# hieunghia-pat/OpenViIC

Hardware: AMD Instinct MI355X
Metric: captions/sec (whole node) at beam=5, 50 regions x d2048 (higher is better)
Workload: dtype f32; 1 GPU; standard_transformer beam=5, B=256 per GPU, 50x2048 synthetic regions, V=10201, max_len=20, random-init weights; global_batch=256, parallelism=dp1, streams=4

## Files before the change

### openviic_amd/csrc/gemm.hip

```cpp
#include <atomic>
#include <type_traits>
#include <mutex>
#include <vector>

#include <hip/hip_ext.h>

#include "common.h"
#include "dropout.h"

namespace {


#ifndef OVC_F32_BUFS
#define OVC_F32_BUFS 1
#endif
template <int BM, int BN, int WM, int WN, int WK, int BK, int NC>
struct TileConfig {
    static constexpr int LDT = BK + 4;
    static constexpr int kThreads = 256;
    static constexpr int kWaveM = BM / WM;
    static constexpr int kWaveN = BN / WN;
    static constexpr int TM = kWaveM / 32;
    static constexpr int TN = kWaveN / 32;
    static constexpr int kLoadA = BM * (BK / 4) / kThreads;
    static constexpr int kLoadB = BN * (BK / 4) / kThreads;
    static constexpr int kChains = NC * WK;
    static constexpr int kBufs = OVC_F32_BUFS;
    static constexpr int kTileFloats = kBufs * (BM + BN) * LDT;
    static constexpr int kRedFloats = (WK - 1) * NC * BM * BN;
    static constexpr int kLdsFloats = kTileFloats > kRedFloats ? kTileFloats : kRedFloats;
    static_assert(WM * WN * WK == 4, "four waves per workgroup");
    static_assert(kChains == 1 || kChains == 4, "K-order classes: one chain or four");
    static_assert(BK % 8 == 0 && (kChains == 1 || BK % 32 == 0), "a K tile holds whole 8-deep groups (four chains: whole 4-group periods)");
    static_assert(kWaveM % 32 == 0 && kWaveN % 32 == 0, "wave tile must be a multiple of 32x32");
    static_assert(kLoadA >= 1 && kLoadB >= 1, "tile too small for 256 loader threads");

};

__device__ __forceinline__ int xcd_remap(int bid, int nwg) {
    const int xcd = bid & 7, q = nwg >> 3, r = nwg & 7;
    const int base = xcd < r ? xcd * (q + 1) : r * (q + 1) + (xcd - r) * q;
    return base + (bid >> 3);
}

__device__ __forceinline__ void tile_coords(int tiles_m, int group_m, int xcd_pm, int& tile_m, int& tile_n_all) {
    const int nwg = gridDim.x;
    const int tile = xcd_remap(blockIdx.x, nwg);
    const int tiles_n_all = nwg / tiles_m;
    if (xcd_pm > 0) {
        const int per_chunk = nwg >> 3, chunk = tile / per_chunk, j = tile - chunk * per_chunk;
        const int sub_m = tiles_m / xcd_pm, cm = chunk % xcd_pm, cn = chunk / xcd_pm;
        const int sub_n = tiles_n_all / (8 / xcd_pm);
        tile_m = cm * sub_m + j % sub_m;
        tile_n_all = cn * sub_n + j / sub_m;
    } else {
        const int group_size = group_m * tiles_n_all;
        const int group = tile / group_size;
        const int first_m = group * group_m;
        const int gm = min(group_m, tiles_m - first_m);
        const int in_group = tile - group * group_size;
        tile_n_all = in_group / gm;
        tile_m = first_m + (in_group - tile_n_all * gm);
    }
}

struct TileMap {
    int nwg, tiles_m, tiles_n_all, tiles_n_per_seg;
    int xcd_pm, pm_shift, sub_m, sub_n;
    unsigned sub_m_magic, seg_magic;
    int group_m, group_size, gm_last;
    unsigned group_size_magic, group_m_magic, gm_last_magic;
    int kslice;
};

__device__ __forceinline__ int fast_div(int x, unsigned magic, int d) {
    if (d == 1) return x;
    const unsigned q = __umulhi((unsigned)x, magic);
    return (int)(q * (unsigned)d > (unsigned)x ? q - 1 : q);
}

__device__ __forceinline__ void tile_coords_fast(const TileMap& t, int bid, int& tile_m, int& tile_n_all) {
    const int xcd = bid & 7, q = t.nwg >> 3, r = t.nwg & 7;
    if (t.xcd_pm > 0) {
        const int j = bid >> 3;
        const int cm = xcd & (t.xcd_pm - 1), cn = xcd >> t.pm_shift;
        const int jq = fast_div(j, t.sub_m_magic, t.sub_m);
        tile_m = cm * t.sub_m + (j - jq * t.sub_m);
        tile_n_all = cn * t.sub_n + jq;
    } else {
        const int base = xcd < r ? xcd * (q + 1) : r * (q + 1) + (xcd - r) * q;
        const int tile = base + (bid >> 3);
        const int group = fast_div(tile, t.group_size_magic, t.group_size);
        const int first_m = group * t.group_m;
        const int in_group = tile - group * t.group_size;
        const bool last = first_m + t.group_m > t.tiles_m;
        const int gm = last ? t.gm_last : t.group_m;
        tile_n_all = last ? fast_div(in_group, t.gm_last_magic, t.gm_last) : fast_div(in_group, t.group_m_magic, t.group_m);
        tile_m = first_m + (in_group - tile_n_all * gm);
    }
}

template <int TM, int TN, bool kDrop = false>
__device__ __forceinline__ void store_wave_tiles(const GemmArgs& p, const float* __restrict__ bias, float* __restrict__ Cseg,
                                                 const f32x16 (&acc)[TM][TN], int m0, int n0, int lane,
                                                 const DropoutSite& drop = DropoutSite{}) {
    float* __restrict__ C = Cseg + (size_t)blockIdx.y * p.part_stride;
    uint64_t drop_seed = 0;
    if constexpr (kDrop) drop_seed = (uint64_t)*drop.seed;
    const int half = lane >> 5;
    const bool has_res = p.R != nullptr;
    const __amdgpu_buffer_rsrc_t rsrc_c = __builtin_amdgcn_make_buffer_rsrc(C, 0, p.M * p.ldc * 4, 0x00020000);
    const __amdgpu_buffer_rsrc_t rsrc_r = __builtin_amdgcn_make_buffer_rsrc(const_cast<float*>(has_res ? p.R : p.A1), 0,
                                                                             has_res && p.res_mod == 0 ? p.M * p.ldr * 4 : 0, 0x00020000);
    constexpr int kOutOfRange = 0x7ffffff0;
#pragma unroll
    for (int j = 0; j < TN; ++j) {
        const int n = n0 + j * 32 + (lane & 31);
        const bool n_ok = n < p.seg_n;
        const float bv = bias ? bias[min(n, p.seg_n - 1)] : 0.f;
#pragma unroll
        for (int i = 0; i < TM; ++i) {
            const int mbase = m0 + i * 32 + 4 * half;
            float out[16];
#pragma unroll
            for (int r = 0; r < 16; ++r) {
                const float v = acc[i][j][r] + bv;
                out[r] = p.act == 1 ? fmaxf(v, 0.f) : v;
            }
            if constexpr (kDrop) {
                uint32_t keep = 0;
#pragma unroll 1
                for (int r = 0; r < 16; ++r) {
                    const uint64_t row = (uint64_t)(mbase + (r & 3) + 8 * (r >> 2));
                    keep |= (ovc_dropout_keep(drop_seed, drop.site, row * (uint64_t)drop.cols + (uint64_t)n, drop.thr) ? 1u : 0u) << r;
                }
#pragma unroll
                for (int r = 0; r < 16; ++r) out[r] = (keep >> r) & 1u ? out[r] * drop.scale : 0.f;
            }
            if (has_res) {
                float res[16];
                if (p.res_mod == 0) {
                    const int voff_r = n_ok ? (mbase * p.ldr + n) * 4 : kOutOfRange;
#pragma unroll
                    for (int r = 0; r < 16; ++r)
                        res[r] = __builtin_bit_cast(float, __builtin_amdgcn_raw_buffer_load_b32(rsrc_r, voff_r, ((r & 3) + 8 * (r >> 2)) * p.ldr * 4, 0));
                } else {
#pragma unroll
                    for (int r = 0; r < 16; ++r) {
                        const int mc = min(mbase + (r & 3) + 8 * (r >> 2), p.M - 1) % p.res_mod;
                        res[r] = p.R[(size_t)mc * p.ldr + min(n, p.seg_n - 1)];
                    }
                }
#pragma unroll
                for (int r = 0; r < 16; ++r) out[r] += res[r];
            }
            const int voff_c = n_ok ? (mbase * p.ldc + n) * 4 : kOutOfRange;
#pragma unroll
            for (int r = 0; r < 16; ++r)
                __builtin_amdgcn_raw_buffer_store_b32(__builtin_bit_cast(int, out[r]), rsrc_c, voff_c, ((r & 3) + 8 * (r >> 2)) * p.ldc * 4, 0);
            if (p.stats_t) {
                const int mrow = m0 + i * 32 + 4 * half;
                float v[16];
                float bm = -INFINITY;
#pragma unroll
                for (int r = 0; r < 16; ++r) {
                    v[r] = mrow + (r & 3) + 8 * (r >> 2) < p.M ? out[r] : -INFINITY;
                    bm = fmaxf(bm, v[r]);
                }
                float x, y;
                ovc_swap_rows<true>(bm, x, y);
                bm = fmaxf(x, y);
                float bs = 0.f;
#pragma unroll
                for (int r = 0; r < 16; ++r) bs += __expf(v[r] - bm);
                ovc_swap_rows<true>(bs, x, y);
                bs = x + y;
                if (lane < 32 && n_ok && m0 + i * 32 < p.M)
                    *reinterpret_cast<f32x2*>(p.stats_t + 2 * ((size_t)n * p.stats_ld + ((m0 + i * 32) >> 5))) = f32x2{bm, bs};
            }
            if (p.stats) {
                float bm = 0.f, bs = 0.f;
#pragma unroll
                for (int r = 0; r < 16; ++r) {
                    const float v = n_ok ? out[r] : -INFINITY;
                    const float m = half_wave_max(v);
                    const float sum = half_wave_sum(__expf(v - m));
                    if ((lane & 15) == r) { bm = m; bs = sum; }
                }
                const int rr = lane & 15, row = mbase + (rr & 3) + 8 * (rr >> 2);
                if ((lane & 31) < 16 && row < p.M && n0 + j * 32 < p.seg_n)
                    *reinterpret_cast<f32x2*>(p.stats + 2 * ((size_t)row * p.stats_ld + ((n0 + j * 32) >> 5))) = f32x2{bm, bs};
            }
        }
    }
}

template <int TM, int TN>
__device__ __forceinline__ void store_wave_tiles_score(const GemmArgs& p, const float* __restrict__ bias, const f32x16 (&acc)[TM][TN],
                                                       int m0, int n0, int lane, const int32_t* __restrict__ tgt,
                                                       float* __restrict__ tgt_logit) {
    const int half = lane >> 5;
#pragma unroll
    for (int j = 0; j < TN; ++j) {
        const int n = n0 + j * 32 + (lane & 31);
        const bool n_ok = n < p.seg_n;
        const float bv = bias ? bias[min(n, p.seg_n - 1)] : 0.f;
        const int target = n_ok ? tgt[n] : -1;
#pragma unroll
        for (int i = 0; i < TM; ++i) {
            const int mbase = m0 + i * 32 + 4 * half;
            float out[16];
#pragma unroll
            for (int r = 0; r < 16; ++r) {
                const float v = acc[i][j][r] + bv;
                out[r] = p.act == 1 ? fmaxf(v, 0.f) : v;
            }
#pragma unroll
            for (int r = 0; r < 16; ++r)
                if (target - mbase == (r & 3) + 8 * (r >> 2)) tgt_logit[n] = out[r];
            const int mrow = m0 + i * 32 + 4 * half;
            float v[16];
            float bm = -INFINITY;
#pragma unroll
            for (int r = 0; r < 16; ++r) {
                v[r] = mrow + (r & 3) + 8 * (r >> 2) < p.M ? out[r] : -INFINITY;
                bm = fmaxf(bm, v[r]);
            }
            float x, y;
            ovc_swap_rows<true>(bm, x, y);
            bm = fmaxf(x, y);
            float bs = 0.f;
#pragma unroll
            for (int r = 0; r < 16; ++r) bs += __expf(v[r] - bm);
            ovc_swap_rows<true>(bs, x, y);
            bs = x + y;
            if (lane < 32 && n_ok && m0 + i * 32 < p.M)
                *reinterpret_cast<f32x2*>(p.stats_t + 2 * ((size_t)n * p.stats_ld + ((m0 + i * 32) >> 5))) = f32x2{bm, bs};
        }
    }
}

#include "gemm_split.h"
#include "gemm_rows16.h"

template <int BM, int BN, int BK, int NC>
constexpr int min_waves_per_simd() { return BM * BN <= 32 * 64 ? 5 : (BM * BN <= 64 * 64 ? (NC == 4 && BK == 64 ? 3 : 4) : 1); }

template <int BM, int BN, int WM, int WN, int WK, int BK, int NC>
__global__ __launch_bounds__(256, (min_waves_per_simd<BM, BN, BK, NC>())) void gemm_f32_mfma(TileMap tmap, GemmArgs p) {
#define OVC_GEMM_F32_EPILOGUE \
    store_wave_tiles<Cfg::TM, Cfg::TN>(p, seg_bias, seg_C, acc[0], m0 + wm * Cfg::kWaveM, n0 + wn * Cfg::kWaveN, lane)
#include "gemm_f32_body.inc"
#undef OVC_GEMM_F32_EPILOGUE
}

template <int BM, int BN, int WM, int WN, int WK, int BK, int NC>
__global__ __launch_bounds__(256, (min_waves_per_simd<BM, BN, BK, NC>())) void gemm_f32_mfma_gated(TileMap tmap, GemmArgs p,
                                                                                                 const int32_t* __restrict__ gate) {
    if (ovc_gate_closed(gate)) return;
#define OVC_GEMM_F32_EPILOGUE \
    store_wave_tiles<Cfg::TM, Cfg::TN>(p, seg_bias, seg_C, acc[0], m0 + wm * Cfg::kWaveM, n0 + wn * Cfg::kWaveN, lane)
#include "gemm_f32_body.inc"
#undef OVC_GEMM_F32_EPILOGUE
}

template <int BM, int BN, int WM, int WN, int WK, int BK, int NC>
__global__ __launch_bounds__(256, (min_waves_per_simd<BM, BN, BK, NC>())) void gemm_f32_mfma_dropout(TileMap tmap, GemmArgs p,
                                                                                                   DropoutSite drop) {
#define OVC_GEMM_F32_EPILOGUE \
    store_wave_tiles<Cfg::TM, Cfg::TN, true>(p, seg_bias, seg_C, acc[0], m0 + wm * Cfg::kWaveM, n0 + wn * Cfg::kWaveN, lane, drop)
#include "gemm_f32_body.inc"
#undef OVC_GEMM_F32_EPILOGUE
}

template <int BM, int BN, int WM, int WN, int WK, int BK, int NC>
__global__ __launch_bounds__(256, (min_waves_per_simd<BM, BN, BK, NC>())) void gemm_f32_mfma_score(TileMap tmap, GemmArgs p,
                                                                                                 const int32_t* tgt, float* tgt_logit) {
#define OVC_GEMM_F32_EPILOGUE \
    store_wave_tiles_score<Cfg::TM, Cfg::TN>(p, seg_bias, acc[0], m0 + wm * Cfg::kWaveM, n0 + wn * Cfg::kWaveN, lane, tgt, tgt_logit)
#include "gemm_f32_body.inc"
#undef OVC_GEMM_F32_EPILOGUE
}

enum TileOrderRegime { kOrderSuperRows = 0, kOrderSplitSmallA = 1, kOrderSplitLargeA = 2 };
int tile_order(const GemmArgs& a, int tiles_m, int tiles_n, int* group_m, int* xcd_pm) {
    const size_t a_bytes = sizeof(float) * (size_t)a.M * (a.K1 + a.K2);
    *group_m = a_bytes <= (size_t)3 << 20 ? tiles_m : (tiles_m < 8 ? tiles_m : 8);
    *xcd_pm = 0;
    const int slices = a.ksplit > 1 ? a.ksplit : 1;
    const size_t w_bytes = sizeof(float) * (size_t)a.seg_n * a.nseg * (a.K1 + a.K2);
    const int tiles_n_all = tiles_n * a.nseg;
    if (a_bytes / slices <= (size_t)3 << 20) {
        size_t best = 8 * a_bytes + w_bytes;
        for (int pm = 2; pm <= 8; pm *= 2) {
            if (tiles_m % pm || tiles_n_all % (8 / pm)) continue;
            const size_t cost = (size_t)(8 / pm) * a_bytes + (size_t)pm * w_bytes;
            if (cost < best) { best = cost; *xcd_pm = pm; }
        }
        if (*xcd_pm > 0) return kOrderSplitSmallA;
    } else if (slices == 1 && w_bytes <= (size_t)3 << 20) {
        size_t best = ~(size_t)0;
        for (int pm = 8; pm >= 2; pm /= 2) {
            if (tiles_m % pm || tiles_n_all % (8 / pm) || a_bytes / pm > (size_t)3 << 20) continue;
            const size_t cost = (size_t)(8 / pm) * a_bytes + (size_t)pm * w_bytes;
            if (cost < best) { best = cost; *xcd_pm = pm; }
        }
        if (*xcd_pm > 0) return kOrderSplitLargeA;
    }
    return kOrderSuperRows;
}

inline void tile_counts(const GemmArgs& a, int bm, int bn, int* tiles_m, int* tiles_n) {
    *tiles_m = (a.M + bm - 1) / bm;
    *tiles_n = (a.seg_n + bn - 1) / bn;
}

enum GemmInstance { kInstPlain = 0, kInstGated = 1, kInstDropout = 2, kInstScoring = 3, kInstPlanesDirect = 4 };
inline int f32_instance(const GemmLaunchOpts& opts) {
    return opts.tgt_logit ? kInstScoring : (opts.drop_seed ? kInstDropout : (opts.gate ? kInstGated : kInstPlain));
}
inline bool split_reads_planes(const GemmArgs& a, int bk) {
    bool planes = (a.K1 + a.K2) % bk == 0 && a.K1 % bk == 0;
    for (int s = 0; s < a.nseg; ++s) planes = planes && a.seg[s].Wp != nullptr;
    return planes;
}

TileMap make_tile_map(int nwg, int tiles_m, int tiles_n_per_seg, int group_m, int xcd_pm, int kslice) {
    auto magic = [](int d) { return d > 1 ? (unsigned)(((uint64_t)1 << 32) / (uint64_t)d + 1) : 0u; };
    TileMap t{};
    t.nwg = nwg; t.tiles_m = tiles_m; t.tiles_n_all = nwg / tiles_m; t.tiles_n_per_seg = tiles_n_per_seg;
// ... 613 lines not shown
```

### openviic_amd/csrc/gemm_f32_body.inc

```
    using Cfg = TileConfig<BM, BN, WM, WN, WK, BK, NC>;
    constexpr int LDT = Cfg::LDT;
    constexpr int kVecPerRow = BK / 4;
    constexpr int kRowsPerPass = 256 / kVecPerRow;
    extern __shared__ __attribute__((aligned(16))) float lds[];

    const int tid = threadIdx.x;
    const int lane = tid & 63;
    const int wave = tid >> 6;
    const int wk = wave / (WM * WN);
    const int wm = (wave / WN) % WM, wn = wave % WN;

    const TileMap t = tmap;
    const float* const a1_ptr = p.A1;
    const float* const w0_ptr = p.seg[0].W;
    const float* const bias0_ptr = p.seg[0].bias;
    float* const c0_ptr = p.seg[0].C;
    const float* const a2_shared = p.A2;
    uint8_t* const zero_rows_ptr = p.zero_rows_out;
    const int arg_lda1 = p.lda1, arg_lda2 = p.lda2, arg_K1 = p.K1, arg_K2 = p.K2, arg_M = p.M, arg_seg_n = p.seg_n, arg_nseg = p.nseg;
    asm volatile("" ::"s"(t.nwg), "s"(t.tiles_m), "s"(t.tiles_n_all), "s"(t.tiles_n_per_seg), "s"(t.xcd_pm), "s"(t.pm_shift), "s"(t.sub_m),
                 "s"(t.sub_n), "s"(t.sub_m_magic), "s"(t.seg_magic), "s"(t.group_m), "s"(t.group_size), "s"(t.gm_last),
                 "s"(t.group_size_magic), "s"(t.group_m_magic), "s"(t.gm_last_magic), "s"(t.kslice), "s"(a1_ptr), "s"(w0_ptr),
                 "s"(bias0_ptr), "s"(c0_ptr), "s"(arg_lda1), "s"(arg_K1), "s"(arg_K2), "s"(arg_M), "s"(arg_seg_n), "s"(arg_nseg),
                 "s"(a2_shared), "s"(zero_rows_ptr), "s"(arg_lda2), "s"(p.R), "s"(p.ldc), "s"(p.ldr), "s"(p.res_mod), "s"(p.act),
                 "s"(p.part_stride), "s"(p.stats), "s"(p.stats_t), "s"(p.stats_ld));

    int tile_m, tile_n_all;
    tile_coords_fast(t, (int)blockIdx.x, tile_m, tile_n_all);
    const int seg = arg_nseg == 1 ? 0 : fast_div(tile_n_all, t.seg_magic, t.tiles_n_per_seg);
    const int tile_n = tile_n_all - seg * t.tiles_n_per_seg;
    const int m0 = tile_m * BM, n0 = tile_n * BN;

    const float* __restrict__ W = arg_nseg == 1 ? w0_ptr : p.seg[seg].W;
    const float* __restrict__ seg_bias = arg_nseg == 1 ? bias0_ptr : p.seg[seg].bias;
    float* __restrict__ seg_C = arg_nseg == 1 ? c0_ptr : p.seg[seg].C;
    const int K = arg_K1 + arg_K2;
    const int kslice = t.kslice;
    const int kbase = (int)blockIdx.y * kslice;
    const int nkt = (kslice + BK - 1) / BK;

    constexpr int kBufFloats = (BM + BN) * LDT;

    f32x4 stage_a[Cfg::kLoadA], stage_b[Cfg::kLoadB];

    const bool k_tail = (K % BK) != 0 || (p.K1 % BK) != 0;
    bool a_ok = true, w_ok = true;

    const __amdgpu_buffer_rsrc_t rsrc_a1 = __builtin_amdgcn_make_buffer_rsrc(const_cast<float*>(a1_ptr), 0, arg_M * arg_lda1 * 4, 0x00020000);
    const float* a2 = arg_K2 ? (p.seg[seg].A2 ? p.seg[seg].A2 : a2_shared) : a1_ptr;
    const __amdgpu_buffer_rsrc_t rsrc_a2 = __builtin_amdgcn_make_buffer_rsrc(const_cast<float*>(a2), 0,
                                                                              arg_K2 ? arg_M * arg_lda2 * 4 : 0, 0x00020000);
    const __amdgpu_buffer_rsrc_t rsrc_w = __builtin_amdgcn_make_buffer_rsrc(const_cast<float*>(W), 0, arg_seg_n * K * 4, 0x00020000);
    int off_a1[Cfg::kLoadA], off_a2[Cfg::kLoadA], off_w[Cfg::kLoadB];
    {
        const int kq = tid % kVecPerRow;
#pragma unroll
        for (int i = 0; i < Cfg::kLoadA; ++i) {
            const int row = m0 + tid / kVecPerRow + i * kRowsPerPass;
            off_a1[i] = (row * arg_lda1 + kq * 4) * 4;
            off_a2[i] = (row * arg_lda2 + kq * 4) * 4;
        }
#pragma unroll
        for (int i = 0; i < Cfg::kLoadB; ++i) off_w[i] = ((n0 + tid / kVecPerRow + i * kRowsPerPass) * K + kq * 4) * 4;
    }
    auto load_tile = [&](int kt) {
        const int k0 = kbase + kt * BK;
        const bool second = k0 >= p.K1;
        if (k_tail) {
            const int kq = tid % kVecPerRow;
            a_ok = (second ? k0 - p.K1 : k0) + kq * 4 < (second ? p.K2 : p.K1);
            w_ok = k0 + kq * 4 < K;
        }
        if (!second) {
#pragma unroll
            for (int i = 0; i < Cfg::kLoadA; ++i)
                stage_a[i] = __builtin_bit_cast(f32x4, __builtin_amdgcn_raw_buffer_load_b128(rsrc_a1, off_a1[i], k0 * 4, 0));
        } else {
#pragma unroll
            for (int i = 0; i < Cfg::kLoadA; ++i)
                stage_a[i] = __builtin_bit_cast(f32x4, __builtin_amdgcn_raw_buffer_load_b128(rsrc_a2, off_a2[i], (k0 - p.K1) * 4, 0));
        }
#pragma unroll
        for (int i = 0; i < Cfg::kLoadB; ++i)
            stage_b[i] = __builtin_bit_cast(f32x4, __builtin_amdgcn_raw_buffer_load_b128(rsrc_w, off_w[i], k0 * 4, 0));
    };
    const bool row_sums = zero_rows_ptr != nullptr && tile_n_all == 0;
    float rs[Cfg::kLoadA];
#pragma unroll
    for (int i = 0; i < Cfg::kLoadA; ++i) rs[i] = 0.f;
    auto store_tile = [&](int buf) {
        const int kq = tid % kVecPerRow;
        if (k_tail) {
#pragma unroll
            for (int i = 0; i < Cfg::kLoadA; ++i)
                if (!a_ok) stage_a[i] = f32x4{0.f, 0.f, 0.f, 0.f};
#pragma unroll
            for (int i = 0; i < Cfg::kLoadB; ++i)
                if (!w_ok) stage_b[i] = f32x4{0.f, 0.f, 0.f, 0.f};
        }
        if (row_sums) {
#pragma unroll
            for (int i = 0; i < Cfg::kLoadA; ++i) rs[i] += (stage_a[i][0] + stage_a[i][1]) + (stage_a[i][2] + stage_a[i][3]);
        }
#pragma unroll
        for (int i = 0; i < Cfg::kLoadA; ++i) {
            const int row = tid / kVecPerRow + i * kRowsPerPass;
            *reinterpret_cast<f32x4*>(lds + buf * kBufFloats + row * LDT + kq * 4) = stage_a[i];
        }
#pragma unroll
        for (int i = 0; i < Cfg::kLoadB; ++i) {
            const int row = tid / kVecPerRow + i * kRowsPerPass;
            *reinterpret_cast<f32x4*>(lds + buf * kBufFloats + (BM + row) * LDT + kq * 4) = stage_b[i];
        }
    };

    f32x16 acc[NC][Cfg::TM][Cfg::TN];
#pragma unroll
    for (int c = 0; c < NC; ++c)
#pragma unroll
        for (int i = 0; i < Cfg::TM; ++i)
#pragma unroll
            for (int j = 0; j < Cfg::TN; ++j)
#pragma unroll
                for (int r = 0; r < 16; ++r) acc[c][i][j][r] = 0.f;

    const int frag_row = lane & 31;
    const int frag_k = (lane >> 5) * 4;

    auto compute_tile = [&](int buf) {
        const float* a_base = lds + buf * kBufFloats + (wm * Cfg::kWaveM + frag_row) * LDT + frag_k;
        const float* b_base = lds + buf * kBufFloats + (BM + wn * Cfg::kWaveN + frag_row) * LDT + frag_k;
        constexpr int kGroupsPerWave = Cfg::kChains == 1 ? BK / 8 : (BK / 32) * NC;
#pragma unroll
        for (int g = 0; g < kGroupsPerWave; ++g) {
            const int set = Cfg::kChains == 1 ? 0 : g % NC;
            const int kk = Cfg::kChains == 1 ? g : 4 * (g / NC) + wk + WK * (g % NC);
            f32x4 a[Cfg::TM], b[Cfg::TN];
#pragma unroll
            for (int i = 0; i < Cfg::TM; ++i)
                a[i] = *reinterpret_cast<const f32x4*>(a_base + i * 32 * LDT + kk * 8);
#pragma unroll
            for (int j = 0; j < Cfg::TN; ++j)
                b[j] = *reinterpret_cast<const f32x4*>(b_base + j * 32 * LDT + kk * 8);
            __builtin_amdgcn_s_setprio(1);
#pragma unroll
            for (int s = 0; s < 4; ++s)
#pragma unroll
                for (int i = 0; i < Cfg::TM; ++i)
#pragma unroll
                    for (int j = 0; j < Cfg::TN; ++j)
                        acc[set][i][j] = __builtin_amdgcn_mfma_f32_32x32x2f32(a[i][s], b[j][s], acc[set][i][j], 0, 0, 0);
            __builtin_amdgcn_s_setprio(0);
        }
    };

#ifdef OVC_NO_PF2
    constexpr bool kPF2 = false;
#else
    constexpr bool kPF2 = BM * BN <= 64 * 64 && Cfg::kBufs == 1 && !(WK == 2 && BK == 64);
#endif
    constexpr int kDepth = 2;
    bool done = false;
    if constexpr (kPF2) {
        if (!k_tail && p.K2 == 0 && !row_sums && nkt >= kDepth) {
            f32x4 sa[kDepth][Cfg::kLoadA], sb[kDepth][Cfg::kLoadB];
            auto load_set = [&](int kt, auto set_tag) {
                constexpr int S = decltype(set_tag)::value;
                const int k0 = kbase + kt * BK;
#pragma unroll
                for (int i = 0; i < Cfg::kLoadA; ++i)
                    sa[S][i] = __builtin_bit_cast(f32x4, __builtin_amdgcn_raw_buffer_load_b128(rsrc_a1, off_a1[i], k0 * 4, 0));
#pragma unroll
                for (int i = 0; i < Cfg::kLoadB; ++i)
                    sb[S][i] = __builtin_bit_cast(f32x4, __builtin_amdgcn_raw_buffer_load_b128(rsrc_w, off_w[i], k0 * 4, 0));
            };
            auto store_set = [&](auto set_tag) {
                constexpr int S = decltype(set_tag)::value;
                const int kq = tid % kVecPerRow;
#pragma unroll
                for (int i = 0; i < Cfg::kLoadA; ++i)
                    *reinterpret_cast<f32x4*>(lds + (tid / kVecPerRow + i * kRowsPerPass) * LDT + kq * 4) = sa[S][i];
#pragma unroll
                for (int i = 0; i < Cfg::kLoadB; ++i)
                    *reinterpret_cast<f32x4*>(lds + (BM + tid / kVecPerRow + i * kRowsPerPass) * LDT + kq * 4) = sb[S][i];
            };
            auto step = [&](int kt, auto cur_tag) {
                constexpr int C = decltype(cur_tag)::value;
                if (kt + kDepth < nkt) load_set(kt + kDepth, cur_tag);
                compute_tile(0);
                if (kt + 1 < nkt) {
                    __syncthreads();
                    store_set(std::integral_constant<int, (C + 1) % kDepth>{});
                    __syncthreads();
                }
            };
            load_set(0, std::integral_constant<int, 0>{});
            if constexpr (kDepth > 1) load_set(1, std::integral_constant<int, 1 % kDepth>{});
            if constexpr (kDepth > 2) load_set(2, std::integral_constant<int, 2 % kDepth>{});
            if constexpr (kDepth > 3) load_set(3, std::integral_constant<int, 3 % kDepth>{});
            store_set(std::integral_constant<int, 0>{});
            __syncthreads();
            for (int kt = 0; kt < nkt; kt += kDepth) {
                step(kt, std::integral_constant<int, 0>{});
                if constexpr (kDepth > 1) { if (kt + 1 < nkt) step(kt + 1, std::integral_constant<int, 1 % kDepth>{}); }
                if constexpr (kDepth > 2) { if (kt + 2 < nkt) step(kt + 2, std::integral_constant<int, 2 % kDepth>{}); }
                if constexpr (kDepth > 3) { if (kt + 3 < nkt) step(kt + 3, std::integral_constant<int, 3 % kDepth>{}); }
            }
            __syncthreads();
            done = true;
        }
    }
    if (!done) {
        load_tile(0);
        store_tile(0);
        __syncthreads();
        for (int kt = 0; kt < nkt; ++kt) {
            const int buf = Cfg::kBufs == 2 ? (kt & 1) : 0;
            if (kt + 1 < nkt) load_tile(kt + 1);
            compute_tile(buf);
            if (kt + 1 < nkt) {
                if (Cfg::kBufs == 1) __syncthreads();
                store_tile(Cfg::kBufs == 2 ? (buf ^ 1) : 0);
            }
            __syncthreads();
        }
    }

    if (row_sums) {
#pragma unroll
        for (int i = 0; i < Cfg::kLoadA; ++i) {
            float v = rs[i];
#pragma unroll
            for (int off = 1; off < kVecPerRow; off <<= 1) v += __shfl_xor(v, off, 64);
            const int row = m0 + tid / kVecPerRow + i * kRowsPerPass;
            if (tid % kVecPerRow == 0 && row < arg_M) zero_rows_ptr[row] = (v == 0.f) ? 1 : 0;
        }
    }

    if (Cfg::kChains > 1) {
        float* red = lds;
        const int wtile = wm * WN + wn;
        auto red_index = [&](int w, int c, int i, int j, int r) {
            return ((((((w - 1) * NC + c) * (WM * WN) + wtile) * Cfg::TM + i) * Cfg::TN + j) * 16 + r) * 64 + lane;
        };
        if (WK > 1) {
            if (wk > 0) {
#pragma unroll
                for (int c = 0; c < NC; ++c)
#pragma unroll
                    for (int i = 0; i < Cfg::TM; ++i)
#pragma unroll
                        for (int j = 0; j < Cfg::TN; ++j)
#pragma unroll
                            for (int r = 0; r < 16; ++r) red[red_index(wk, c, i, j, r)] = acc[c][i][j][r];
            }
            __syncthreads();
            if (wk > 0) return;
        }
#pragma unroll
        for (int chain = 1; chain < Cfg::kChains; ++chain) {
            constexpr int kW = WK;
            const int w = chain % kW, c = chain / kW;
#pragma unroll
            for (int i = 0; i < Cfg::TM; ++i)
#pragma unroll
                for (int j = 0; j < Cfg::TN; ++j)
#pragma unroll
                    for (int r = 0; r < 16; ++r)
                        acc[0][i][j][r] += w == 0 ? acc[c][i][j][r] : red[red_index(w, c, i, j, r)];
        }
    }

    OVC_GEMM_F32_EPILOGUE;
```

Measured before the change: 21600 captions/s.

## Double-buffer LDS in small f32 GEMM tiles and interleave stores with MFMAs

For four-chain, BK=32, small-tile f32 GEMM configs, the prefetch path now uses two LDS buffers. It writes the next K tile's staged registers into the alternate buffer, spread between the MFMAs of the current tile, and register-prefetches the next LDS fragment group. This removes one of the two barriers per K step and hides LDS write latency behind matrix math. In exchange it doubles LDS use for those configs, which may lower occupancy. It also forces instruction order with sched_barriers, which may constrain the compiler.

```diff
diff --git a/openviic_amd/csrc/gemm.hip b/openviic_amd/csrc/gemm.hip
--- a/openviic_amd/csrc/gemm.hip
+++ b/openviic_amd/csrc/gemm.hip
@@ -13,6 +13,11 @@
 
 #ifndef OVC_F32_BUFS
 #define OVC_F32_BUFS 1
+#endif
+#ifdef OVC_NO_LDS2
+#define OVC_F32_LDS2 0
+#else
+#define OVC_F32_LDS2 1
 #endif
 template <int BM, int BN, int WM, int WN, int WK, int BK, int NC>
 struct TileConfig {
@@ -25,7 +30,8 @@
     static constexpr int kLoadA = BM * (BK / 4) / kThreads;
     static constexpr int kLoadB = BN * (BK / 4) / kThreads;
     static constexpr int kChains = NC * WK;
-    static constexpr int kBufs = OVC_F32_BUFS;
+    static constexpr bool kLds2 = OVC_F32_LDS2 && kChains == 4 && BK == 32 && BM * BN <= 64 * 64;
+    static constexpr int kBufs = kLds2 ? 2 : OVC_F32_BUFS;
     static constexpr int kTileFloats = kBufs * (BM + BN) * LDT;
     static constexpr int kRedFloats = (WK - 1) * NC * BM * BN;
     static constexpr int kLdsFloats = kTileFloats > kRedFloats ? kTileFloats : kRedFloats;
diff --git a/openviic_amd/csrc/gemm_f32_body.inc b/openviic_amd/csrc/gemm_f32_body.inc
--- a/openviic_amd/csrc/gemm_f32_body.inc
+++ b/openviic_amd/csrc/gemm_f32_body.inc
@@ -157,8 +157,9 @@
 #ifdef OVC_NO_PF2
     constexpr bool kPF2 = false;
 #else
-    constexpr bool kPF2 = BM * BN <= 64 * 64 && Cfg::kBufs == 1 && !(WK == 2 && BK == 64);
+    constexpr bool kPF2 = BM * BN <= 64 * 64 && (Cfg::kBufs == 1 || Cfg::kLds2) && !(WK == 2 && BK == 64);
 #endif
+    constexpr bool kLDS2 = kPF2 && Cfg::kLds2;
     constexpr int kDepth = 2;
     bool done = false;
     if constexpr (kPF2) {
@@ -174,15 +175,15 @@
                 for (int i = 0; i < Cfg::kLoadB; ++i)
                     sb[S][i] = __builtin_bit_cast(f32x4, __builtin_amdgcn_raw_buffer_load_b128(rsrc_w, off_w[i], k0 * 4, 0));
             };
+            float* const stage_dst = lds + (tid / kVecPerRow) * LDT + (tid % kVecPerRow) * 4;
+            auto store_one = [&](auto set_tag, int w, int buf) {
+                constexpr int S = decltype(set_tag)::value;
+                const int row = w < Cfg::kLoadA ? w * kRowsPerPass : BM + (w - Cfg::kLoadA) * kRowsPerPass;
+                *reinterpret_cast<f32x4*>(stage_dst + buf * kBufFloats + row * LDT) = w < Cfg::kLoadA ? sa[S][w] : sb[S][w - Cfg::kLoadA];
+            };
             auto store_set = [&](auto set_tag) {
-                constexpr int S = decltype(set_tag)::value;
-                const int kq = tid % kVecPerRow;
-#pragma unroll
-                for (int i = 0; i < Cfg::kLoadA; ++i)
-                    *reinterpret_cast<f32x4*>(lds + (tid / kVecPerRow + i * kRowsPerPass) * LDT + kq * 4) = sa[S][i];
-#pragma unroll
-                for (int i = 0; i < Cfg::kLoadB; ++i)
-                    *reinterpret_cast<f32x4*>(lds + (BM + tid / kVecPerRow + i * kRowsPerPass) * LDT + kq * 4) = sb[S][i];
+#pragma unroll
+                for (int w = 0; w < Cfg::kLoadA + Cfg::kLoadB; ++w) store_one(set_tag, w, 0);
             };
             auto step = [&](int kt, auto cur_tag) {
                 constexpr int C = decltype(cur_tag)::value;
@@ -194,19 +195,84 @@
                     __syncthreads();
                 }
             };
+            auto load_set_if = [&](int kt, bool live, auto set_tag) {
+                constexpr int S = decltype(set_tag)::value;
+                const int k0 = kbase + kt * BK;
+                const __amdgpu_buffer_rsrc_t ra = __builtin_amdgcn_make_buffer_rsrc(const_cast<float*>(a1_ptr), 0, live ? arg_M * arg_lda1 * 4 : 0, 0x00020000);
+                const __amdgpu_buffer_rsrc_t rw = __builtin_amdgcn_make_buffer_rsrc(const_cast<float*>(W), 0, live ? arg_seg_n * K * 4 : 0, 0x00020000);
+#pragma unroll
+                for (int i = 0; i < Cfg::kLoadA; ++i)
+                    sa[S][i] = __builtin_bit_cast(f32x4, __builtin_amdgcn_raw_buffer_load_b128(ra, off_a1[i], k0 * 4, 0));
+#pragma unroll
+                for (int i = 0; i < Cfg::kLoadB; ++i)
+                    sb[S][i] = __builtin_bit_cast(f32x4, __builtin_amdgcn_raw_buffer_load_b128(rw, off_w[i], k0 * 4, 0));
+            };
+            auto step2 = [&](int kt, auto cur_tag) {
+                constexpr int C = decltype(cur_tag)::value;
+                constexpr int kGroups = (BK / 32) * NC;
+                constexpr int kMfmas = kGroups * 4 * Cfg::TM * Cfg::TN, kWrites = Cfg::kLoadA + Cfg::kLoadB;
+                constexpr int kEvery = kMfmas / kWrites;
+                static_assert(kEvery >= 1, "more LDS writes than MFMAs in a K tile");
+                load_set_if(kt + kDepth, kt + kDepth < nkt, cur_tag);
+                const float* a_base = lds + C * kBufFloats + (wm * Cfg::kWaveM + frag_row) * LDT + frag_k;
+                const float* b_base = lds + C * kBufFloats + (BM + wn * Cfg::kWaveN + frag_row) * LDT + frag_k;
+                f32x4 fa[2][Cfg::TM], fb[2][Cfg::TN];
+                auto read_group = [&](int g) {
+                    const int kk = 4 * (g / NC) + wk + WK * (g % NC);
+#pragma unroll
+                    for (int i = 0; i < Cfg::TM; ++i) fa[g & 1][i] = *reinterpret_cast<const f32x4*>(a_base + i * 32 * LDT + kk * 8);
+#pragma unroll
+                    for (int j = 0; j < Cfg::TN; ++j) fb[g & 1][j] = *reinterpret_cast<const f32x4*>(b_base + j * 32 * LDT + kk * 8);
+                };
+                read_group(0);
+#pragma unroll
+                for (int g = 0; g < kGroups; ++g) {
+                    __builtin_amdgcn_sched_barrier(0);
+                    __builtin_amdgcn_s_setprio(1);
+#pragma unroll
+                    for (int s = 0; s < 4; ++s)
+#pragma unroll
+                        for (int i = 0; i < Cfg::TM; ++i)
+#pragma unroll
+                            for (int j = 0; j < Cfg::TN; ++j) {
+                                acc[g % NC][i][j] = __builtin_amdgcn_mfma_f32_32x32x2f32(fa[g & 1][i][s], fb[g & 1][j][s], acc[g % NC][i][j], 0, 0, 0);
+                                const int m = ((g * 4 + s) * Cfg::TM + i) * Cfg::TN + j;
+                                if (m % kEvery == 0 && m / kEvery < kWrites) {
+                                    __builtin_amdgcn_sched_barrier(0);
+                                    store_one(std::integral_constant<int, (C + 1) % kDepth>{}, m / kEvery, C ^ 1);
+                                    __builtin_amdgcn_sched_barrier(0);
+                                }
+                                if (s == 0 && i == Cfg::TM - 1 && j == Cfg::TN - 1 && g + 1 < kGroups) {
+                                    read_group(g + 1);
+                                    __builtin_amdgcn_sched_barrier(0);
+                                }
+                            }
+                    __builtin_amdgcn_s_setprio(0);
+                    __builtin_amdgcn_sched_barrier(0);
+                }
+                __syncthreads();
+            };
             load_set(0, std::integral_constant<int, 0>{});
             if constexpr (kDepth > 1) load_set(1, std::integral_constant<int, 1 % kDepth>{});
             if constexpr (kDepth > 2) load_set(2, std::integral_constant<int, 2 % kDepth>{});
             if constexpr (kDepth > 3) load_set(3, std::integral_constant<int, 3 % kDepth>{});
             store_set(std::integral_constant<int, 0>{});
             __syncthreads();
-            for (int kt = 0; kt < nkt; kt += kDepth) {
-                step(kt, std::integral_constant<int, 0>{});
-                if constexpr (kDepth > 1) { if (kt + 1 < nkt) step(kt + 1, std::integral_constant<int, 1 % kDepth>{}); }
-                if constexpr (kDepth > 2) { if (kt + 2 < nkt) step(kt + 2, std::integral_constant<int, 2 % kDepth>{}); }
-                if constexpr (kDepth > 3) { if (kt + 3 < nkt) step(kt + 3, std::integral_constant<int, 3 % kDepth>{}); }
+            if constexpr (kLDS2) {
+                static_assert(kDepth == 2, "LDS buffer and register set of a tile are both its index & 1");
+                for (int kt = 0; kt < nkt; kt += 2) {
+                    step2(kt, std::integral_constant<int, 0>{});
+                    if (kt + 1 < nkt) step2(kt + 1, std::integral_constant<int, 1>{});
+                }
+            } else {
+                for (int kt = 0; kt < nkt; kt += kDepth) {
+                    step(kt, std::integral_constant<int, 0>{});
+                    if constexpr (kDepth > 1) { if (kt + 1 < nkt) step(kt + 1, std::integral_constant<int, 1 % kDepth>{}); }
+                    if constexpr (kDepth > 2) { if (kt + 2 < nkt) step(kt + 2, std::integral_constant<int, 2 % kDepth>{}); }
+                    if constexpr (kDepth > 3) { if (kt + 3 < nkt) step(kt + 3, std::integral_constant<int, 3 % kDepth>{}); }
+                }
+                __syncthreads();
             }
-            __syncthreads();
             done = true;
         }
     }
@@ -214,13 +280,14 @@
         load_tile(0);
         store_tile(0);
         __syncthreads();
+        constexpr int kPlainBufs = Cfg::kLds2 ? 1 : Cfg::kBufs;
         for (int kt = 0; kt < nkt; ++kt) {
-            const int buf = Cfg::kBufs == 2 ? (kt & 1) : 0;
+            const int buf = kPlainBufs == 2 ? (kt & 1) : 0;
             if (kt + 1 < nkt) load_tile(kt + 1);
             compute_tile(buf);
             if (kt + 1 < nkt) {
-                if (Cfg::kBufs == 1) __syncthreads();
-                store_tile(Cfg::kBufs == 2 ? (buf ^ 1) : 0);
+                if (kPlainBufs == 1) __syncthreads();
+                store_tile(kPlainBufs == 2 ? (buf ^ 1) : 0);
             }
             __syncthreads();
         }
```

Result: no change. 21510 captions/s (-0.4%).
